# LeiXu84/fireFoam-dev

Measured on AMD Instinct MI355X. Metric: PIMPLE outer-iterations/sec on 64M-cell hex mesh; pEqn SpMV GB/s vs HBM peak, higher is better.
Workload: dtype f64; 1 GPU; synthetic 400^3 hex box (64000000 cells), buoyant plume + 5-species EDC-shaped source, PIMPLE 1/2/0: rhoEqn + UEqn + YEEqn(4 Yi + h) + 2 pEqn per step; cells=64000000, faces=191520000, parallelism=1 GPU, transport_solvers=PBiCGStab+DILU

## Files before the change

firefoam-dev_amd/binding.py:

```python
import ctypes as C
import os
import re
import subprocess

import numpy as np

_HERE = os.path.dirname(os.path.abspath(__file__))
_ROOT = os.path.dirname(_HERE)
_SO = os.path.join(_HERE, "lib", "libffm.so")
_HDR = os.path.join(_ROOT, "include", "ffm.h")

SOLVERS = {"PCG": 0, "PBiCGStab": 1, "PBiCG": 2, "diagonal": 3, "smoothSolver": 4}
PRECONDS = {"none": 0, "DIC": 1, "DILU": 2, "GaussSeidel": 3, "symGaussSeidel": 4, "diagonal": 5}


class FfmError(RuntimeError):
    pass


class Perf(C.Structure):
    _fields_ = [("initialResidual", C.c_double), ("finalResidual", C.c_double),
                ("nIterations", C.c_int), ("converged", C.c_int), ("singular", C.c_int)]

    def as_dict(self):
# ... 69 lines not shown
        "ffm_ldu_bind_coeffs_native_d": ([vp, dp, dp, dp, C.c_int], C.c_int),
        "ffm_ldu_set_interfaces": ([vp, C.c_int, ip, C.POINTER(ip), C.POINTER(hp), C.POINTER(hp), ip], C.c_int),
        "ffm_ldu_set_global_cells": ([vp, C.c_long], C.c_int),
        "ffm_ldu_global_cells": ([vp], C.c_long),
        "ffm_spmv": ([vp, dp, dp], C.c_int),
        "ffm_tmul": ([vp, dp, dp], C.c_int),
        "ffm_sumA": ([vp, dp], C.c_int),
        "ffm_residual": ([vp, dp, dp, dp], C.c_int),
        "ffm_precond_setup": ([vp, C.c_int, dp], C.c_int),
        "ffm_precond_apply": ([vp, C.c_int, C.c_int, dp, dp], C.c_int),
        "ffm_precond_setup_multi": ([vp, C.c_int, C.c_int, C.POINTER(C.c_void_p), C.POINTER(C.c_void_p)], C.c_int),
        "ffm_ldu_tile_reach": ([vp, C.POINTER(C.c_int), C.POINTER(C.c_int), C.POINTER(C.c_int)], C.c_int),
        "ffm_gs_smooth": ([vp, C.c_int, C.c_int, dp, dp], C.c_int),
        "ffm_solve_d": ([vp, C.c_int, C.c_int, C.c_double, C.c_double, C.c_int, C.c_int, C.c_int, dp, dp,
                         C.POINTER(Perf)], C.c_int),
        "ffm_solve": ([vp, C.c_int, C.c_int, C.c_double, C.c_double, C.c_int, C.c_int, C.c_int, hp, hp,
                       C.POINTER(Perf)], C.c_int),
        "ffm_solve_multi_d": ([vp, C.c_int, C.c_int, C.c_int, C.c_double, C.c_double, C.c_int, C.c_int, C.POINTER(C.c_void_p), dp, dp,
                               C.POINTER(C.c_void_p), C.POINTER(C.c_void_p), C.POINTER(Perf)], C.c_int),
        "ffm_ldu_unbind_coeffs": ([vp], C.c_int),
        "ffm_ldu_offdiag_epoch": ([vp], C.c_ulong),
        "ffm_ldu_tile_coef_read": ([vp, C.c_int, hp], C.c_int),
        "ffm_ldu_tile_gathers": ([vp], C.c_long),
        "ffm_debug_pool_poison": ([vp, C.c_int], C.c_int),
        "ffm_bench_spmv": ([vp, dp, dp, C.c_int, hp], C.c_int),
        "ffm_bench_precond": ([vp, C.c_int, dp, dp, C.c_int, hp], C.c_int),
        "ffm_debug_set_sweep_ticket": ([vp, C.c_uint], C.c_int),
        "ffm_ldu_set_exchange_tags": ([vp, C.c_int, C.c_int, ip], C.c_int),
        "ffm_field_binary": ([vp, C.c_int, C.c_long, dp, dp, dp], C.c_int),
        "ffm_field_scalar": ([vp, C.c_int, C.c_long, dp, C.c_double, C.c_int, dp], C.c_int),
        "ffm_field_unary": ([vp, C.c_int, C.c_long, dp, dp], C.c_int),
        "ffm_field_eval": ([vp, C.c_long, C.c_int, C.POINTER(C.c_void_p), C.c_int, hp, C.c_int, C.POINTER(C.c_ushort), dp], C.c_int),
        "ffm_reduce_sum": ([vp, dp, C.c_long, hp], C.c_int),
        "ffm_reduce_min": ([vp, dp, C.c_long, hp], C.c_int),
        "ffm_reduce_max": ([vp, dp, C.c_long, hp], C.c_int),
        "ffm_reduce_dot": ([vp, dp, dp, C.c_long, hp], C.c_int),
        "ffm_reduce_summag": ([vp, dp, C.c_long, hp], C.c_int),
        "ffm_mesh_create": ([vp, hp, hp, hp, hp, hp, hp, C.c_int, ip, C.POINTER(ip), C.POINTER(hp), C.POINTER(hp), C.POINTER(vp)], C.c_int),
        "ffm_mesh_destroy": ([vp], C.c_int),
        "ffm_mesh_set_face_centres": ([vp, hp], C.c_int),
        "ffm_mesh_set_nonorth_correction": ([vp, hp], C.c_int),
        "ffm_pyro_create": ([vp, C.c_int, C.c_int, C.c_double, C.c_double, C.c_double, C.c_double, C.POINTER(vp)], C.c_int),
        "ffm_pyro_set_solids": ([vp, hp, hp], C.c_int),
        "ffm_pyro_set_reaction": ([vp, C.c_double, C.c_double, C.c_double, C.c_double], C.c_int),
        "ffm_pyro_step": ([vp, C.c_double, dp, C.c_int, C.c_double], C.c_int),
        "ffm_pyro_get": ([vp, C.c_char_p, hp], C.c_int),
# ... 484 lines not shown
        return m

    def bind_coeffs_native(self, diag, upper, lower=None, offDiagUnchanged=False):
        self._bound = (diag, upper, lower)
        _check(lib().ffm_ldu_bind_coeffs_native_d(self.h, C.c_void_p(diag.data_ptr()), C.c_void_p(upper.data_ptr()),
                                                  None if lower is None else C.c_void_p(lower.data_ptr()), 1 if offDiagUnchanged else 0),
               "ffm_ldu_bind_coeffs_native_d")
        return self

    def unbind_coeffs(self):
        _check(lib().ffm_ldu_unbind_coeffs(self.h), "ffm_ldu_unbind_coeffs")
        self._bound = None
        return self

    def tile_coef(self, which):
        self.ctx._ready()
        out = np.empty(3 * self.nOwned, np.float64)
        _check(lib().ffm_ldu_tile_coef_read(self.h, which, _hp(out)), "ffm_ldu_tile_coef_read")
        return out

    def tile_gathers(self):
        return int(lib().ffm_ldu_tile_gathers(self.h))

    @property
    def offdiag_epoch(self):
        return int(lib().ffm_ldu_offdiag_epoch(self.h))

    def debug_set_sweep_ticket(self, value):
        _check(lib().ffm_debug_set_sweep_ticket(self.h, int(value) & 0xFFFFFFFF), "ffm_debug_set_sweep_ticket")

    @property
    def native_order(self):
        return bool(lib().ffm_ldu_is_native_order(self.h))

    def cell_order(self):
        o = np.empty(self.nCells, np.int32)
        _check(lib().ffm_ldu_get_cell_order(self.h, _ip(o)), "ffm_ldu_get_cell_order")
        return o

    def set_coeffs(self, diag, upper, lower=None):
        T = self.ctx.torch
        if T.is_tensor(diag):
            self.ctx._ready()
            lo = None if lower is None else C.c_void_p(lower.data_ptr())
            _check(lib().ffm_ldu_set_coeffs_d(self.h, C.c_void_p(diag.data_ptr()), C.c_void_p(upper.data_ptr()), lo),
                   "ffm_ldu_set_coeffs_d")
# ... 574 lines not shown
```

firefoam-dev_amd/csrc/ffm_host.hpp:

```cpp
#pragma once
#include <ctime>
#include <cstdio>
#include <cstdlib>
#include <cstring>
#include <vector>
#include <thread>
#include <algorithm>

#include "../../include/ffm.h"

void ffm_set_error(const char *fmt, ...);

#define FFM_TRY(call)                                                            \
    do {                                                                         \
        int r_ = (call);                                                         \
        if (r_ != FFM_OK) return r_;                                             \
    } while (0)

template <class Fn> inline void ffm_parallel_for(long n, Fn fn, long serialBelow = 1L << 20)
{
    static const int nT = [] { const char *e = getenv("FFM_HOST_THREADS"); int t = e ? atoi(e) : (int)std::thread::hardware_concurrency(); return std::max(1, std::min(t, 16)); }();
    if (n < serialBelow || nT == 1) { fn(0L, n); return; }
    std::vector<std::thread> th;
    const long chunk = (n + nT - 1) / nT;
// ... 24 lines not shown
    std::vector<int> newToOldCell, oldToNewCell, newToOldFace;
    std::vector<int> l, u;
    std::vector<int> fwdLevelStart;
    std::vector<int> bwdLevelStart;
    std::vector<int> bwdOrder;
    bool identity = true;
    int mode = 0, nGroups = 0; bool bwdIsReverse = false;
    std::vector<int> levNew, blNew;
    std::vector<int> grpCell;
};
struct LduLayout {
    int nSlices = 0, upTotal = 0, loTotal = 0;
    int upWidthUniform = -1, loWidthUniform = -1, maxW = 0;
    int loShift = 4;
    std::vector<int> upOff, loOff;
    std::vector<int> upNbr, faceSrc;
    std::vector<int> loEnt;
    std::vector<int> callerToNative;
    std::vector<int> rowSched;
};
int ffm_ldu_analysis(int nOwn, int nGhost, int F, const int *l, const int *u, const int *groupHint, int forceMode, LduAnalysis &a);
int ffm_ldu_layout(const LduAnalysis &a, int nOwn, int nGhost, int F, LduLayout &L);
bool ffm_tile_feasible(int nOwn, int F, const int *l, const int *u);
```

firefoam-dev_amd/csrc/ffm_tile.hip:

```cpp
#include "ffm_internal.hpp"
#include "ffm_device.hpp"
#include <algorithm>
#include <atomic>
#include <climits>

constexpr int T_RING = 4096;
constexpr int T_ENT = 256;
constexpr int T_THREADS = 256;
constexpr int T_W = FFM_TILE_W;
constexpr int T_PF = 8;
constexpr int T_PM = 3;
constexpr int T_XMAX = 64;
constexpr int T_RINGD = T_RING - 2 * T_ENT;
constexpr unsigned T_SPIN_LIMIT = 1u << 22;
constexpr unsigned T_NONE = 0xFFFFu;
constexpr int T_LDS = T_RING + 2 * T_XMAX + 1;
constexpr unsigned long long T_SENT = 0x7FF4DEADBEEFCAFEull;
static_assert(T_LDS < (int)T_NONE && T_ENT <= 256, "neighbour codes are LDS slots");
static_assert(T_PM >= 2 && T_PM < T_PF, "read-ahead distances");

struct TileDir {
    int nEnt = 0, nPub = 0;
    int *grpEnt = nullptr;
    int4 *rec = nullptr;
    int *extSrc = nullptr;
    unsigned short *code = nullptr;
    int *src = nullptr;
    double *coefU = nullptr, *coefL = nullptr;
    unsigned long epochU = ~0ul, epochL = ~0ul;
    int reach = 0;
    double *mail = nullptr;
};

struct ffm_tile_plan {
    bool usable = false;
    int G = 0;
    TileDir f, b;
    double *mailAll = nullptr;
    long nMail = 0;
    double *mailMulti = nullptr;
    bool amulUsable = false;
    bool gsTables = false;
    std::vector<int> grpEntHost;
    int4 *arec = nullptr;
    uint4 *acode = nullptr;
    int2 *aext = nullptr;
    int *upNbrCell = nullptr;
    int nSeg = 0;
    int4 *aseg = nullptr;
    double *amulPartials = nullptr;
    int4 *fvSeg = nullptr; int nFvSeg = 0, fvRun = 0;
    int nTail = 0;
    int *tailCell = nullptr, *tailStart = nullptr, *tailFace = nullptr, *tailNbr = nullptr;
};

bool ffm_tile_fv_segments(ffm_ldu *A, int runLength, FfmFvSegs *out)
{
    ffm_tile_plan *T = A->tile;
    if (!T || !T->usable || T->grpEntHost.empty() || A->nCells != A->nOwned) return false;
    if (!T->fvSeg || T->fvRun != runLength) {
        std::vector<int4> seg;
        const std::vector<int> &ge = T->grpEntHost;
        for (int g = 0; g < T->G; g++) for (int a = ge[g]; a < ge[g + 1]; a += runLength) seg.push_back(make_int4(ge[g], a, std::min(a + runLength, ge[g + 1]), ge[g + 1]));
        if (T->fvSeg) { hipFree(T->fvSeg); T->fvSeg = nullptr; }
        if (ffm_upload_vec(A->ctx, &T->fvSeg, seg) != FFM_OK) return false;
        T->nFvSeg = (int)seg.size(); T->fvRun = runLength;
    }
    out->nSeg = T->nFvSeg; out->seg = T->fvSeg; out->rec = T->f.rec;
    return true;
}

static void free_dir(TileDir &d)
{
    hipFree(d.grpEnt); hipFree(d.rec); hipFree(d.extSrc); hipFree(d.code); hipFree(d.src); hipFree(d.coefU); hipFree(d.coefL);
    d = TileDir();
}
void ffm_tile_free(ffm_ldu *A)
{
    if (!A->tile) return;
    free_dir(A->tile->f); free_dir(A->tile->b);
    hipFree(A->tile->mailAll); hipFree(A->tile->mailMulti);
    hipFree(A->tile->arec); hipFree(A->tile->acode); hipFree(A->tile->aext); hipFree(A->tile->aseg); hipFree(A->tile->amulPartials);
    hipFree(A->tile->fvSeg); hipFree(A->tile->upNbrCell);
    hipFree(A->tile->tailCell); hipFree(A->tile->tailStart); hipFree(A->tile->tailFace); hipFree(A->tile->tailNbr);
    delete A->tile; A->tile = nullptr;
}
bool ffm_tile_usable(const ffm_ldu *A) { return A->tile && A->tile->usable; }

template <class T> static int upv(ffm_ctx *c, T **d, const std::vector<T> &v) { return ffm_upload_vec(c, d, v); }

static int build_dir(ffm_ldu *A, bool fwd, const std::vector<int> &lvl, const std::vector<int> &grpCell,
                     const std::vector<int> &grpOfCell, TileDir &D, bool &ok, std::vector<int4> *recOut = nullptr,
                     std::vector<int> *grpEntOut = nullptr)
{
    const int G = (int)grpCell.size() - 1, nOwn = A->nOwned, W = T_W, sh = A->loShift;
    const std::vector<int> &off = fwd ? A->h_loOff : A->h_upOff;
    const std::vector<int> &ent = fwd ? A->h_loEnt : A->h_upNbr;
    std::vector<int> nbr((size_t)W * nOwn, -1), src((size_t)W * nOwn, -1);
    std::vector<unsigned char> exposed(nOwn, 0);
    auto isExt = [&](int c, int nb) { return grpOfCell[nb] != grpOfCell[c] || std::abs(c - nb) > T_RINGD; };
    std::atomic<int> tooMany(0), reach(0);
    ffm_parallel_for(nOwn, [&](long c0_, long c1_) {
        int far = 0;
        for (long c = c0_; c < c1_; c++) {
            const int sl = (int)(c >> 6), lane = (int)(c & 63), wdt = (off[sl + 1] - off[sl]) / 64;
            int k = 0;
            for (int s = 0; s < wdt; s++) {
                const int q = off[sl] + s * 64 + lane, e = ent[q];
                if (e < 0) continue;
                const int nb = fwd ? (e >> sh) : e;
                if (nb >= nOwn) continue;
                if (k >= W) { tooMany = 1; break; }
// ... 45 lines not shown
    for (int4 &R : rec) { R.w = (int)nExtAll; nExtAll += (size_t)(R.y >> 16); }
    std::vector<int> extSrc(nExtAll);
    std::atomic<int> bad(0);
    ffm_parallel_for((long)rec.size(), [&](long e0_, long e1_) {
        for (long ei = e0_; ei < e1_; ei++) {
            const int4 &R = rec[ei];
            const int c0 = R.x, cnt = R.y & 0xFFFF;
            const int gs = cnt ? grpCell[grpOfCell[c0]] : 0;
            int t = 0;
            for (int c = c0; c < c0 + cnt; c++) for (int k = 0; k < W; k++) {
                const int nb = nbr[(size_t)W * c + k];
                if (nb < 0) continue;
                if (isExt(c, nb)) {
                    if (mailIdx[nb] < 0 || t >= (R.y >> 16)) { bad = mailIdx[nb] < 0 ? 1 : 2; continue; }
                    code[(size_t)4 * c + k] = (unsigned short)(T_RING + (int)(ei & 1) * T_XMAX + t); extSrc[(size_t)R.w + t] = mailIdx[nb]; t++;
                } else code[(size_t)4 * c + k] = (unsigned short)((nb - gs) & (T_RING - 1));
            }
            if (t != (R.y >> 16)) bad = 2;
        }
    }, nOwn >= (1 << 20) ? 1024 : (1L << 40));
    if (bad == 1) { ffm_set_error("internal: tile plan references an unpublished cell"); return FFM_ERR_ADDR; }
    if (bad) { ffm_set_error("internal: tile plan external count mismatch"); return FFM_ERR_ADDR; }
    D.nEnt = (int)rec.size(); D.nPub = nPub;
    if (recOut) *recOut = rec;
    if (grpEntOut) *grpEntOut = grpEnt;
    for (int k = 0; k < 2 * T_PF + 2; k++) rec.push_back(make_int4(0, 0, 0, 0));
    for (int k = 0; k < T_THREADS; k++) extSrc.push_back(0);
    FFM_TRY(upv(A->ctx, &D.grpEnt, grpEnt)); FFM_TRY(upv(A->ctx, &D.rec, rec)); FFM_TRY(upv(A->ctx, &D.extSrc, extSrc)); FFM_TRY(upv(A->ctx, &D.code, code)); FFM_TRY(upv(A->ctx, &D.src, src));
    return FFM_OK;
}

constexpr int A_RING = 1024;
constexpr int A_WIN = 1;
constexpr int A_AHEAD = A_WIN + 1;
constexpr int A_XMAX = 128;
constexpr int A_PF = 6;
constexpr unsigned A_NONE = 0xFFFFu, A_EXT = 0x8000u;
static_assert((A_WIN + A_AHEAD + 1) * T_ENT <= A_RING && A_PF > A_AHEAD, "ring window");

static int build_amul(ffm_ldu *A, const std::vector<int> &grpOfCell, const std::vector<int4> &recF)
{
    ffm_tile_plan *T = A->tile;
    const int nOwn = A->nOwned, nEnt = (int)recF.size();
    std::vector<int> tailCell, tailStart(1, 0), tailFace, tailNbr;
    std::vector<int> upNb((size_t)3 * nOwn, -1);
    for (int c = 0; c < nOwn; c++) {
        const int sl = c >> 6, lane = c & 63;
        const int uw = (A->h_upOff[sl + 1] - A->h_upOff[sl]) / 64;
        int k = 0;
        bool ghostSeen = false;
        for (int s = 0; s < uw; s++) {
// ... 35 lines not shown
                const int o = q >> A->loShift, os = q & ((1 << A->loShift) - 1);
                if (k >= 3) { AMUL_GIVE_UP("more than 3 lower neighbours"); }
                if (inRing(c, o) && os < 3 && c - o < 2048) code[(size_t)8 * c + k] = (unsigned short)((c - o) | (os << 12));
                else {
                    if (t >= A_XMAX) { AMUL_GIVE_UP("more than A_XMAX externals in one entry"); }
                    code[(size_t)8 * c + k] = (unsigned short)(A_EXT | t);
                    aext.push_back(make_int2(o, A->h_upOff[o >> 6] + os * 64 + (o & 63))); t++;
                }
                k++;
            }
            for (k = 0; k < 3; k++) {
                const int nb = upNb[(size_t)3 * c + k];
                if (nb < 0) break;
                if (inRing(c, nb) && nb - c < 2048) code[(size_t)8 * c + 3 + k] = (unsigned short)(nb - c);
                else {
                    if (t >= A_XMAX) { AMUL_GIVE_UP("more than A_XMAX externals in one entry"); }
                    code[(size_t)8 * c + 3 + k] = (unsigned short)(A_EXT | t);
                    aext.push_back(make_int2(nb, -1)); t++;
                }
            }
        }
        arec[e] = make_int4(c0, cnt | (t << 16), extOff, 0);
    }
    for (int k = 0; k < 2 * A_PF + 2; k++) arec.push_back(make_int4(0, 0, 0, 0));
    for (int k = 0; k < 2 * A_XMAX; k++) aext.push_back(make_int2(0, -1));
    FFM_TRY(upv(A->ctx, &T->arec, arec)); FFM_TRY(upv(A->ctx, &T->aext, aext));
    FFM_HIP(hipMalloc((void **)&T->acode, sizeof(unsigned short) * 8 * std::max<size_t>(nOwn, 1)));
    FFM_TRY(ffm_h2d(A->ctx, T->acode, code.data(), sizeof(unsigned short) * code.size()));
    {
        const std::vector<int> &grpEntH = T->grpEntHost;
        const int L = std::min(20, std::max(16, nEnt / 2048));
        std::vector<int4> seg;
        for (int g = 0; g < T->G; g++) for (int a = grpEntH[g]; a < grpEntH[g + 1]; a += L) seg.push_back(make_int4(g, a, std::min(a + L, grpEntH[g + 1]), grpEntH[g + 1]));
        T->nSeg = (int)seg.size();
        FFM_TRY(upv(A->ctx, &T->aseg, seg));
        FFM_HIP(hipMalloc((void **)&T->amulPartials, sizeof(double) * std::max(T->nSeg, 1)));
    }
    T->amulUsable = true;
    return FFM_OK;
}

int ffm_tile_build(ffm_ldu *A, const std::vector<int> &lev, const std::vector<int> &bl, const std::vector<int> &grpCell)
{
    A->tile = new ffm_tile_plan();
    ffm_tile_plan *T = A->tile;
    T->G = (int)grpCell.size() - 1;
    if (T->G <= 0) return FFM_OK;
    const int nOwn = A->nOwned;
    if ((long)A->nCells * 24 >= (1L << 32)) return FFM_OK;
    std::vector<int> grpOfCell(nOwn);
    for (int g = 0; g < T->G; g++) for (int c = grpCell[g]; c < grpCell[g + 1]; c++) grpOfCell[c] = g;
    bool ok = true;
    std::vector<int4> recF;
    { FfmStageTimer tm_("tile: forward plan"); FFM_TRY(build_dir(A, true, lev, grpCell, grpOfCell, T->f, ok, &recF, &T->grpEntHost)); }
    if (ok) { FfmStageTimer tm_("tile: backward plan"); FFM_TRY(build_dir(A, false, bl, grpCell, grpOfCell, T->b, ok)); }
    T->usable = ok;
    if (ok) {
        T->nMail = (long)T->f.nPub + T->b.nPub + 2;
        FFM_HIP(hipMalloc((void **)&T->mailAll, sizeof(double) * T->nMail));
        T->f.mail = T->mailAll; T->b.mail = T->mailAll + T->f.nPub + 1;
        FfmStageTimer tm_("tile: amul plan");
        FFM_TRY(build_amul(A, grpOfCell, recF));
        if (!T->gsTables) T->usable = false;
    }
    return FFM_OK;
}

struct TileView {
    int G;
    const int *grpCell, *grpEnt, *extSrc;
    const int4 *rec;
    const uint2 *code;
    unsigned int *ticket;
};

__device__ __forceinline__ double t_ld(const double *p) { return __hip_atomic_load(p, __ATOMIC_RELAXED, __HIP_MEMORY_SCOPE_AGENT); }
__device__ __forceinline__ void t_st(double *p, double v) { __hip_atomic_store(p, v, __ATOMIC_RELAXED, __HIP_MEMORY_SCOPE_AGENT); }
__device__ __forceinline__ void t_barrier() { asm volatile("s_waitcnt lgkmcnt(0)\n\ts_barrier" ::: "memory"); }
__device__ __forceinline__ bool t_pending(double v) { return (unsigned long long)__double_as_longlong(v) == T_SENT; }

enum { TM_FWD = 0, TM_BWD = 1, TM_RD = 2, TM_GSF = 3, TM_GSB = 4 };
struct __attribute__((aligned(8))) T3 { double a, b, c; };
static_assert(T_W == 3, "T3");

__device__ __noinline__ double t_wait_value(const double *addr, unsigned int *ticket, int *shAbort)
{
    double v = t_ld(addr);
    if (*(volatile int *)shAbort) return v;
    unsigned spins = 0;
    while (t_pending(v)) {
        __builtin_amdgcn_s_sleep(1);
        v = t_ld(addr);
        if ((++spins & 1023u) == 0u) {
// ... 24 lines not shown
    constexpr bool VEC = MODE != TM_RD;
    constexpr int W = T_W, PF = tile_pf(NF, MODE);
    __shared__ double ring[NF][LDS];
    __shared__ double shSum[4];
    __shared__ int4 shRec[4];
    __shared__ int shG;
    __shared__ int shAbort;
    const unsigned tid = threadIdx.x;
    if (tid == 0) {
        const unsigned tk = atomicAdd(&t.ticket[0], 1u);
        const int k = (int)(tk % (unsigned)t.G);
        shG = ASC ? k : t.G - 1 - k; shAbort = 0;
    }
    __syncthreads();
    const int g = __builtin_amdgcn_readfirstlane(shG);
    const unsigned gs = (unsigned)__builtin_amdgcn_readfirstlane(t.grpCell[g]);
    const int e0 = __builtin_amdgcn_readfirstlane(t.grpEnt[g]), e1 = __builtin_amdgcn_readfirstlane(t.grpEnt[g + 1]);
    if (e0 >= e1) { if (FUSE && tid == 0) partials[g] = 0.0; return; }

    if (tid >= (unsigned)T_THREADS) {
        const unsigned lane = tid - (unsigned)T_THREADS;
        int4 qrec[PF];
        unsigned qne[PF], qxi[PF];
        double qxv[PF][NF];
#define Q_REC(k, e) { qrec[k] = t.rec[min((e), e1)]; }
#define Q_IDX(k, e) { const int4 R_ = qrec[k]; qne[k] = ((e) < e1) ? ((unsigned)R_.y >> 16) : 0u; qxi[k] = (unsigned)t.extSrc[(unsigned)R_.w + (lane < qne[k] ? lane : 0u)]; }
#define Q_MAIL(k) { _Pragma("unroll") for (int i_ = 0; i_ < NF; i_++) qxv[k][i_] = t_ld(&m.mail[i_][lane < qne[k] ? qxi[k] : 0u]); }
#define Q_PUT(k, e) {                                                                                    \
        if (lane < qne[k]) {                                                                              \
            _Pragma("unroll") for (int i_ = 0; i_ < NF; i_++) {                                           \
                double v_ = qxv[k][i_];                                                                   \
                if (__builtin_expect(t_pending(v_), 0)) v_ = t_wait_value(&m.mail[i_][qxi[k]], t.ticket, &shAbort); \
                ring[i_][R + (((e) & 1) * T_XMAX) + lane] = v_;                                           \
            }                                                                                             \
        }                                                                                                 \
    }
#pragma unroll
        for (int k = 0; k < PF; k++) Q_REC(k, e0 + k);
#pragma unroll
        for (int k = 0; k < PF; k++) { Q_IDX(k, e0 + k); Q_REC(k, e0 + PF + k); }
#pragma unroll
        for (int k = 0; k < T_PM; k++) Q_MAIL(k);
        Q_PUT(0, e0);
        if (lane == 0) shRec[(e0 + PF) & 3] = qrec[0];
        t_barrier();
        for (int e = e0; e < e1; e += PF) {
#pragma unroll
            for (int k = 0; k < PF; k++) {
                const int ee = e + k;
// ... 2 lines not shown
                Q_IDX(k, ee + PF);
                Q_REC(k, ee + 2 * PF);
                Q_MAIL((k + T_PM) % PF);
                t_barrier();
            }
        }
#undef Q_REC
#undef Q_IDX
#undef Q_MAIL
#undef Q_PUT
        return;
    }

    unsigned pc[PF], ppb[PF];
    bool pok[PF];
    uint2 pq[PF];
    double pa[PF][W], pb[PF][TWO ? W : 1], pd[PF][NF], pv[PF][VEC ? NF : 1], pv2[FUSE ? PF : 1];
    double fsum = 0.0;
    const double fAlpha = (FUSE && MODE == TM_FWD) ? scal[S_ALPHA] : 0.0;
    const bool fSing = (FUSE && MODE == TM_FWD) ? (scal[S_SING] != 0.0) : false;
#define T_FETCH(k, e, R_) {                                                                             \
        const unsigned cnt_ = ((e) < e1) ? ((unsigned)R_.y & 0xFFFFu) : 0u;                              \
        const bool ok_ = tid < cnt_;                                                                     \
        const unsigned cc_ = ok_ ? (ASC ? (unsigned)R_.x + tid : (unsigned)R_.x + cnt_ - 1u - tid) : gs; \
        const unsigned o8_ = cc_ * 8u, o24_ = cc_ * 24u;          \
        pq[k] = *(const uint2 *)((const char *)t.code + o8_);                                            \
        { const T3 v_ = *(const T3 *)((const char *)ca + o24_); pa[k][0] = v_.a; pa[k][1] = v_.b; pa[k][2] = v_.c; }     \
        if (TWO) { const T3 v_ = *(const T3 *)((const char *)cb + o24_); pb[k][0] = v_.a; pb[k][TWO ? 1 : 0] = v_.b; pb[k][TWO ? 2 : 0] = v_.c; } \
        _Pragma("unroll") for (int i_ = 0; i_ < NF; i_++) {                                              \
            pd[k][i_] = *(const double *)((const char *)m.dg[i_] + o8_);                                 \
            if (VEC) pv[k][VEC ? i_ : 0] = *(const double *)((const char *)((FUSE && MODE == TM_FWD) ? (const double *)aux : MODE == TM_BWD ? (const double *)m.w[i_] : m.r[i_]) + o8_); \
        }                                                                                                \
        if (FUSE) pv2[FUSE ? k : 0] = *(const double *)((const char *)((MODE == TM_FWD && !m.r[0]) ? (const double *)m.w[0] : m.r[0]) + o8_); \
        pc[k] = cc_; pok[k] = ok_; ppb[k] = (unsigned)R_.z;                                              \
    }
#pragma unroll
    for (int k = 0; k < PF; k++) { const int4 R0 = t.rec[min(e0 + k, e1)]; T_FETCH(k, e0 + k, R0); }
    t_barrier();
    for (int e = e0; e < e1; e += PF) {
#pragma unroll
        for (int k = 0; k < PF; k++) {
            const int ee = e + k;
            const int4 Rn = shRec[(ee + PF) & 3];
            {
                const unsigned c = pc[k];
                const unsigned cd[4] = {pq[k].x & 0xFFFFu, pq[k].x >> 16, pq[k].y & 0xFFFFu, pq[k].y >> 16};
                unsigned sl[W];
#pragma unroll
                for (int s = 0; s < W; s++)
// ... 68 lines not shown
    constexpr int W = T_W;
    constexpr int PF = tile_pf(1, MODE);
    __shared__ double ring[T_LDS];
    double *const halo = ring + T_RING;
    __shared__ int4 shRec[4];
    __shared__ int shG;
    __shared__ int shAbort;
    const unsigned tid = threadIdx.x;
    if (tid == 0) {
        const unsigned tk = atomicAdd(&t.ticket[0], 1u);
        const int k = (int)(tk % (unsigned)t.G);
        shG = ASC ? k : t.G - 1 - k; shAbort = 0;
    }
    __syncthreads();
    const int g = __builtin_amdgcn_readfirstlane(shG);
    const unsigned gs = (unsigned)__builtin_amdgcn_readfirstlane(t.grpCell[g]);
    const int e0 = __builtin_amdgcn_readfirstlane(t.grpEnt[g]), e1 = __builtin_amdgcn_readfirstlane(t.grpEnt[g + 1]);
    if (e0 >= e1) return;

    if (tid >= (unsigned)T_THREADS) {
        const unsigned lane = tid - (unsigned)T_THREADS;
        int4 qrec[PF];
        unsigned qne[PF], qxi[PF];
        double qxv[PF];
#define Q_REC(k, e) { qrec[k] = t.rec[min((e), e1)]; }
#define Q_IDX(k, e) { const int4 R_ = qrec[k]; qne[k] = ((e) < e1) ? ((unsigned)R_.y >> 16) : 0u; qxi[k] = (unsigned)t.extSrc[(unsigned)R_.w + (lane < qne[k] ? lane : 0u)]; }
#define Q_MAIL(k) { qxv[k] = t_ld(&mail[lane < qne[k] ? qxi[k] : 0u]); }
#define Q_PUT(k, e) {                                                                                    \
        if (lane < qne[k]) {                                                                              \
            double v_ = qxv[k];                                                                           \
            if (__builtin_expect(t_pending(v_), 0)) v_ = t_wait_value(&mail[qxi[k]], t.ticket, &shAbort); \
            halo[(((e) & 1) * T_XMAX) + lane] = v_;                                                       \
        }                                                                                                 \
    }
#pragma unroll
        for (int k = 0; k < PF; k++) Q_REC(k, e0 + k);
#pragma unroll
        for (int k = 0; k < PF; k++) { Q_IDX(k, e0 + k); Q_REC(k, e0 + PF + k); }
#pragma unroll
        for (int k = 0; k < T_PM; k++) Q_MAIL(k);
        Q_PUT(0, e0);
        if (lane == 0) shRec[(e0 + PF) & 3] = qrec[0];
        t_barrier();
        for (int e = e0; e < e1; e += PF) {
#pragma unroll
            for (int k = 0; k < PF; k++) {
                const int ee = e + k;
                Q_PUT((k + 1) % PF, ee + 1);
                if (lane == 0) shRec[(ee + 1 + PF) & 3] = qrec[(k + 1) % PF];
                Q_IDX(k, ee + PF);
                Q_REC(k, ee + 2 * PF);
                Q_MAIL((k + T_PM) % PF);
                t_barrier();
            }
        }
#undef Q_REC
#undef Q_IDX
#undef Q_MAIL
#undef Q_PUT
        return;
    }

    unsigned pc[PF], ppb[PF];
    bool pok[PF];
    uint2 pq[PF];
    double pa[PF][W], pb[PF][TWO ? W : 1], pd[PF], pv[PF];
#define T_FETCH(k, e, R_) {                                                                             \
        const unsigned cnt_ = ((e) < e1) ? ((unsigned)R_.y & 0xFFFFu) : 0u;                              \
        const bool ok_ = tid < cnt_;                                                                     \
        const unsigned cc_ = ok_ ? (ASC ? (unsigned)R_.x + tid : (unsigned)R_.x + cnt_ - 1u - tid) : gs; \
        const unsigned o8_ = cc_ * 8u, o24_ = cc_ * 24u;          \
        pq[k] = *(const uint2 *)((const char *)t.code + o8_);                                            \
        { const T3 v_ = *(const T3 *)((const char *)ca + o24_); pa[k][0] = v_.a; pa[k][1] = v_.b; pa[k][2] = v_.c; }     \
        if (TWO) { const T3 v_ = *(const T3 *)((const char *)cb + o24_); pb[k][0] = v_.a; pb[k][TWO ? 1 : 0] = v_.b; pb[k][TWO ? 2 : 0] = v_.c; } \
        pd[k] = *(const double *)((const char *)dg + o8_);                                               \
        pv[k] = *(const double *)((const char *)r + o8_);                                                \
        pc[k] = cc_; pok[k] = ok_; ppb[k] = (unsigned)R_.z;                                              \
    }
#pragma unroll
    for (int k = 0; k < PF; k++) { const int4 R0 = t.rec[min(e0 + k, e1)]; T_FETCH(k, e0 + k, R0); }
    t_barrier();
    for (int e = e0; e < e1; e += PF) {
#pragma unroll
        for (int k = 0; k < PF; k++) {
            const int ee = e + k;
            const int4 Rn = shRec[(ee + PF) & 3];
            {
                const unsigned c = pc[k];
                const unsigned cd[4] = {pq[k].x & 0xFFFFu, pq[k].x >> 16, pq[k].y & 0xFFFFu, pq[k].y >> 16};
                double x[W];
#pragma unroll
                for (int s = 0; s < W; s++) x[s] = ring[min(cd[s], (unsigned)(T_LDS - 1))];
                const double d = pd[k];
                double val;
                if (MODE == TM_GSF) {
// ... 15 lines not shown
            }
            T_FETCH(k, ee + PF, Rn);
            t_barrier();
        }
    }
#undef T_FETCH
}

__global__ void k_tile_gather(long n, const int *__restrict__ src, const double *__restrict__ native, double *__restrict__ out)
{
    for (long i = (long)blockIdx.x * blockDim.x + threadIdx.x; i < n; i += (long)gridDim.x * blockDim.x) {
        const int q = src[i];
        out[i] = (q >= 0) ? native[q] : 0.0;
    }
}
__global__ void k_tile_fill(long n, unsigned long long *p, unsigned long long v, unsigned int *ticket)
{
    if (blockIdx.x == 0 && threadIdx.x == 0) ticket[0] = 0u;
    for (long i = (long)blockIdx.x * blockDim.x + threadIdx.x; i < n; i += (long)gridDim.x * blockDim.x) p[i] = v;
}

static TileView tview(const ffm_ldu *A, const TileDir &d)
{
    TileView t; t.G = A->tile->G; t.grpCell = A->grpCell; t.grpEnt = d.grpEnt; t.extSrc = d.extSrc; t.rec = d.rec;
    t.code = (const uint2 *)d.code; t.ticket = A->sweepTicket;
    return t;
}

static int tile_coef(ffm_ldu *A, TileDir &d, bool upper, const double **out)
{
    const long n = (long)T_W * A->nOwned;
    double *&buf = upper ? d.coefU : d.coefL;
    unsigned long &ep = upper ? d.epochU : d.epochL;
    if (!buf) { FFM_HIP(hipMalloc((void **)&buf, sizeof(double) * std::max<long>(n, 1))); ep = ~0ul; }
    if (ep != A->offDiagEpoch) {
        const int g = std::max(1, std::min(ffm_grid(n, 256), 8 * RED_BLOCKS));
        hipLaunchKernelGGL(k_tile_gather, dim3(g), dim3(256), 0, A->ctx->stream, n, d.src, upper ? A->upper : A->lower, buf);
        ep = A->offDiagEpoch;
        A->tileGathers++;
    }
    *out = buf;
    return FFM_OK;
}

bool ffm_tile_coef_direct_ok(const ffm_ldu *A) { return ffm_tile_usable(A) && A->nCells == A->nOwned && A->maxW <= T_W && A->identity; }
int ffm_tile_coef_direct(ffm_ldu *A, bool lower, double **fU, double **fL, double **bU)
{
// ... 10 lines not shown
    A->directPending = false;
    *fU = T->f.coefU; *fL = lower ? T->f.coefL : nullptr; *bU = T->b.coefU;
    return FFM_OK;
}
void ffm_tile_coef_written(ffm_ldu *A, const double *upper_d, const double *lower_d)
{
    A->directPending = true; A->directUpper = upper_d; A->directLower = (lower_d && lower_d != upper_d) ? lower_d : nullptr;
}
void ffm_tile_coef_adopt(ffm_ldu *A)
{
    ffm_tile_plan *T = A->tile;
    T->f.epochU = T->b.epochU = A->offDiagEpoch;
    if (A->directLower) T->f.epochL = A->offDiagEpoch;
}
extern "C" int ffm_ldu_tile_coef_read(ffm_ldu *A, int which, double *out_h)
{
    if (!A || !out_h || which < 0 || which > 3) return FFM_ERR_ARG;
    if (!ffm_tile_usable(A)) { ffm_set_error("ffm_ldu_tile_coef_read: the matrix has no tile plan"); return FFM_ERR_UNSUPPORTED; }
    const double *p;
    FFM_TRY(tile_coef(A, which < 2 ? A->tile->f : A->tile->b, !(which & 1), &p));
    return ffm_d2h(A->ctx, out_h, p, sizeof(double) * (size_t)T_W * A->nOwned);
}
extern "C" long ffm_ldu_tile_gathers(const ffm_ldu *A) { return A ? (long)A->tileGathers : -1; }

static void tile_fill(ffm_ldu *A, double *p, long n)
{
    const int g = std::max(1, std::min(ffm_grid(n, 256), 8 * RED_BLOCKS));
    hipLaunchKernelGGL(k_tile_fill, dim3(g), dim3(256), 0, A->ctx->stream, n, (unsigned long long *)p, T_SENT, A->sweepTicket);
}

bool ffm_tile_multi_fits(const ffm_ldu *A, int n)
{
    if (n < 1 || n > FFM_TILE_MAXSYS || !ffm_tile_usable(A)) return false;
    return n <= 4 || std::max(A->tile->f.reach, A->tile->b.reach) <= TM_RING5 - 2 * T_ENT;
}
extern "C" int ffm_ldu_tile_reach(const ffm_ldu *A, int *reach, int *limit, int *limit5)
{
    if (!A || !reach || !limit || !limit5) return FFM_ERR_ARG;
    if (!ffm_tile_usable(A)) { ffm_set_error("ffm_ldu_tile_reach: the matrix has no tile plan"); return FFM_ERR_UNSUPPORTED; }
    *reach = std::max(A->tile->f.reach, A->tile->b.reach); *limit = T_RINGD; *limit5 = TM_RING5 - 2 * T_ENT;
    return FFM_OK;
}
static int tile_mail(ffm_ldu *A, int n, bool fwdOnly, double **mail)
{
    ffm_tile_plan *T = A->tile;
    if (n > 1 && !T->mailMulti) FFM_HIP(hipMalloc((void **)&T->mailMulti, sizeof(double) * (size_t)FFM_TILE_MAXSYS * (size_t)T->nMail));
// ... 164 lines not shown
                    if (lane == 0) shRec[(ee + 1 + A_PF) & 3] = qrec[(k + 1) % A_PF];
                    Q_IDX(k, ee + A_PF);
                    Q_REC(k, ee + 2 * A_PF);
                    Q_VAL((k + T_PM) % A_PF);
                    t_barrier();
                }
            }
#undef Q_REC
#undef Q_IDX
#undef Q_VAL
#undef Q_PUT
#undef Q_X0
#undef Q_X1
        } else {
            unsigned pc[A_PF];
            bool pok[A_PF], pst[A_PF];
            uint4 pq[A_PF];
            double pb[A_PF][3], pd[A_PF], px[A_PF], pp[FUSEP ? A_PF : 1], ps[FUSEP ? A_PF : 1], pl[ASYM ? A_PF : 1][3];
#define A_FETCH(k, e, R_) {                                                                              \
        const unsigned cnt_ = ((e) < e1) ? ((unsigned)(R_).y & 0xFFFFu) : 0u;                            \
        const bool ok_ = tid < cnt_;                                                                     \
        const unsigned cc_ = ok_ ? (unsigned)(R_).x + tid : gs;                                          \
        const unsigned o8_ = cc_ * 8u;                                                                   \
        pq[k] = *(const uint4 *)((const char *)t.code + cc_ * 16u);                                      \
        { const T3 v_ = *(const T3 *)((const char *)bc + cc_ * 24u); pb[k][0] = v_.a; pb[k][1] = v_.b; pb[k][2] = v_.c; } \
        pd[k] = *(const double *)((const char *)diag + o8_);                                             \
        px[k] = *(const double *)((const char *)x + o8_);                                                \
        if (FUSEP) { pp[FUSEP ? k : 0] = *(const double *)((const char *)pin + o8_); ps[FUSEP ? k : 0] = *(const double *)((const char *)psi + o8_); } \
        if (ASYM) { const T3 v_ = *(const T3 *)((const char *)lc + cc_ * 24u); pl[ASYM ? k : 0][0] = v_.a; pl[ASYM ? k : 0][1] = v_.b; pl[ASYM ? k : 0][2] = v_.c; } \
        pc[k] = cc_; pok[k] = ok_; pst[k] = ok_ && (e) >= sa && (e) < sb;                                \
    }
#define A_FILL(k) { if (FUSEP) px[k] = fSing ? pp[FUSEP ? k : 0] : px[k] + fBeta * pp[FUSEP ? k : 0];                      \
                    if (pok[k]) { const unsigned i_ = (pc[k] - gs) & (unsigned)(A_RING - 1); xring[i_] = px[k];    \
                                   cring[3u * i_] = pb[k][0]; cring[3u * i_ + 1u] = pb[k][1]; cring[3u * i_ + 2u] = pb[k][2]; } }
#pragma unroll
            for (int k = 0; k < A_PF; k++) { const int4 R0 = t.rec[min(e0 + k, e1)]; A_FETCH(k, e0 + k, R0); }
#pragma unroll
            for (int k = 0; k < A_AHEAD; k++) A_FILL(k);
            t_barrier();
            for (int e = e0; e < sb; e += A_PF) {
#pragma unroll
                for (int k = 0; k < A_PF; k++) {
                    const int ee = e + k;
                    const int4 Rn = shRec[(ee + A_PF) & 3];
                    {
                        const unsigned c = pc[k];
                        const unsigned hb = (unsigned)(ee & 1) * (unsigned)A_XMAX;
// ... 157 lines not shown
```

include/ffm.h:

```cpp
#ifndef FFM_H
#define FFM_H

#include <stddef.h>
#include <stdint.h>

#ifdef __cplusplus
extern "C" {
#endif

typedef struct ffm_ctx ffm_ctx;
typedef struct ffm_ldu ffm_ldu;

typedef enum ffm_status {
    FFM_OK = 0,
    FFM_ERR_ARG = -1,
    FFM_ERR_ADDR = -2,
    FFM_ERR_HIP = -3,
    FFM_ERR_NODEVICE = -4,
    FFM_ERR_UNSUPPORTED = -5,
    FFM_ERR_COMM = -6
} ffm_status;

typedef enum ffm_solver {
    FFM_PCG = 0, FFM_PBICGSTAB = 1, FFM_PBICG = 2, FFM_DIAGONAL = 3, FFM_SMOOTH = 4,
// ... 62 lines not shown
int ffm_ldu_sweep_mode(const ffm_ldu *ldu);
int ffm_ldu_is_native_order(const ffm_ldu *ldu);
int ffm_ldu_get_cell_order(const ffm_ldu *ldu, int *newToOld);

int ffm_renumber_levels(int nCells, int nFaces, const int *lowerAddr,
                        const int *upperAddr, int *newToOldCell,
                        int *newToOldFace);

int ffm_ldu_set_coeffs(ffm_ldu *ldu, const double *diag, const double *upper,
                       const double *lower);
int ffm_ldu_set_coeffs_d(ffm_ldu *ldu, const double *diag_d,
                         const double *upper_d, const double *lower_d);

int ffm_ldu_n_native_faces(const ffm_ldu *ldu);
int ffm_ldu_get_face_map(const ffm_ldu *ldu, int *callerToNative);
int ffm_ldu_set_coeffs_native_d(ffm_ldu *ldu, const double *diag_d,
                                const double *upper_d, const double *lower_d);
int ffm_ldu_bind_coeffs_native_d(ffm_ldu *ldu, const double *diag_d, const double *upper_d,
                                 const double *lower_d, int offDiagUnchanged);
int ffm_ldu_unbind_coeffs(ffm_ldu *ldu);
unsigned long ffm_ldu_offdiag_epoch(const ffm_ldu *ldu);
int ffm_ldu_tile_coef_read(ffm_ldu *ldu, int which, double *out_h);
long ffm_ldu_tile_gathers(const ffm_ldu *ldu);

int ffm_ldu_set_interfaces(ffm_ldu *ldu, int nPatches, const int *patchSizes,
                           const int *const *faceCells,
                           const double *const *bouCoeffs,
                           const double *const *intCoeffs,
                           const int *neighbRank);
int ffm_ldu_set_global_cells(ffm_ldu *ldu, long globalCells);
long ffm_ldu_global_cells(const ffm_ldu *ldu);
int ffm_ldu_set_exchange_tags(ffm_ldu *ldu, int kind, int n, const int *tags);

int ffm_spmv(ffm_ldu *ldu, const double *x_d, double *y_d);
int ffm_tmul(ffm_ldu *ldu, const double *x_d, double *y_d);
int ffm_sumA(ffm_ldu *ldu, double *s_d);
int ffm_residual(ffm_ldu *ldu, const double *x_d, const double *b_d, double *r_d);
int ffm_precond_setup(ffm_ldu *ldu, int precond, double *rD_out_d );
int ffm_precond_apply(ffm_ldu *ldu, int precond, int transpose,
                      const double *r_d, double *w_d);
int ffm_precond_setup_multi(ffm_ldu *ldu, int precond, int nSys, const double *const *diag_d, double *const *rD_out_d);
int ffm_ldu_tile_reach(const ffm_ldu *ldu, int *reach, int *limit, int *limit5);
int ffm_gs_smooth(ffm_ldu *ldu, int symmetric_sweep, int nSweeps, double *psi_d,
                  const double *b_d);

int ffm_solve_d(ffm_ldu *ldu, int solver, int precond, double tolerance,
// ... 365 lines not shown
```

Measured before the change: 3.308 outer-iterations/s.

## Deduplicate per-tile neighbour code blocks into a shared pool

Hashes each tile entry's neighbour-code block at setup and stores identical blocks once in a shared pool, with each record's w field now holding a byte offset into that pool. The external-source offset that used to live in rec.w moves to a separate extOff array. On a structured hex box many tiles have identical connectivity codes, so code reads in the sweep and amul kernels can hit a much smaller, cache-resident footprint. The cost is an extra extOff load per entry, an indirect code address, and host-side hashing at setup; it can be turned off with FFM_TILE_CODE_SHARE.

```diff
diff --git a/firefoam-dev_amd/binding.py b/firefoam-dev_amd/binding.py
--- a/firefoam-dev_amd/binding.py
+++ b/firefoam-dev_amd/binding.py
@@ -115,6 +115,9 @@
         "ffm_ldu_offdiag_epoch": ([vp], C.c_ulong),
         "ffm_ldu_tile_coef_read": ([vp, C.c_int, hp], C.c_int),
         "ffm_ldu_tile_gathers": ([vp], C.c_long),
+        "ffm_ldu_tile_code_bytes": ([vp, C.c_int, C.POINTER(C.c_long), C.POINTER(C.c_long)], C.c_int),
+        "ffm_tile_share_codes": ([C.c_int, C.POINTER(C.c_long), ip, C.POINTER(C.c_ushort), C.c_long, C.c_int, C.c_long, C.POINTER(C.c_uint),
+                                  C.POINTER(C.c_ushort), C.c_long, C.POINTER(C.c_long), C.POINTER(C.c_long)], C.c_int),
         "ffm_debug_pool_poison": ([vp, C.c_int], C.c_int),
         "ffm_bench_spmv": ([vp, dp, dp, C.c_int, hp], C.c_int),
         "ffm_bench_precond": ([vp, C.c_int, dp, dp, C.c_int, hp], C.c_int),
@@ -645,6 +648,11 @@
     def tile_gathers(self):
         return int(lib().ffm_ldu_tile_gathers(self.h))
 
+    def tile_code_bytes(self, which):
+        u, t = C.c_long(), C.c_long()
+        _check(lib().ffm_ldu_tile_code_bytes(self.h, which, C.byref(u), C.byref(t)), "ffm_ldu_tile_code_bytes")
+        return u.value, t.value
+
     @property
     def offdiag_epoch(self):
         return int(lib().ffm_ldu_offdiag_epoch(self.h))
diff --git a/firefoam-dev_amd/csrc/ffm_host.hpp b/firefoam-dev_amd/csrc/ffm_host.hpp
--- a/firefoam-dev_amd/csrc/ffm_host.hpp
+++ b/firefoam-dev_amd/csrc/ffm_host.hpp
@@ -70,3 +70,7 @@
 int ffm_ldu_analysis(int nOwn, int nGhost, int F, const int *l, const int *u, const int *groupHint, int forceMode, LduAnalysis &a);
 int ffm_ldu_layout(const LduAnalysis &a, int nOwn, int nGhost, int F, LduLayout &L);
 bool ffm_tile_feasible(int nOwn, int F, const int *l, const int *u);
+
+int ffm_tile_share(std::vector<unsigned short> &codes, const std::vector<long> &start, const std::vector<int> &len, bool share, long padShorts,
+                   std::vector<unsigned short> &pool, std::vector<unsigned> &off, long *uniqueBytes, long *totalBytes, const char *what);
+bool ffm_tile_share_enabled(int reader);
diff --git a/firefoam-dev_amd/csrc/ffm_tile.hip b/firefoam-dev_amd/csrc/ffm_tile.hip
--- a/firefoam-dev_amd/csrc/ffm_tile.hip
+++ b/firefoam-dev_amd/csrc/ffm_tile.hip
@@ -23,8 +23,10 @@
     int nEnt = 0, nPub = 0;
     int *grpEnt = nullptr;
     int4 *rec = nullptr;
+    int *extOff = nullptr;
     int *extSrc = nullptr;
     unsigned short *code = nullptr;
+    long codeUnique = 0, codeTotal = 0;
     int *src = nullptr;
     double *coefU = nullptr, *coefL = nullptr;
     unsigned long epochU = ~0ul, epochL = ~0ul;
@@ -44,6 +46,7 @@
     std::vector<int> grpEntHost;
     int4 *arec = nullptr;
     uint4 *acode = nullptr;
+    long acodeUnique = 0, acodeTotal = 0;
     int2 *aext = nullptr;
     int *upNbrCell = nullptr;
     int nSeg = 0;
@@ -72,7 +75,7 @@
 
 static void free_dir(TileDir &d)
 {
-    hipFree(d.grpEnt); hipFree(d.rec); hipFree(d.extSrc); hipFree(d.code); hipFree(d.src); hipFree(d.coefU); hipFree(d.coefL);
+    hipFree(d.grpEnt); hipFree(d.rec); hipFree(d.extOff); hipFree(d.extSrc); hipFree(d.code); hipFree(d.src); hipFree(d.coefU); hipFree(d.coefL);
     d = TileDir();
 }
 void ffm_tile_free(ffm_ldu *A)
@@ -88,6 +91,18 @@
 bool ffm_tile_usable(const ffm_ldu *A) { return A->tile && A->tile->usable; }
 
 template <class T> static int upv(ffm_ctx *c, T **d, const std::vector<T> &v) { return ffm_upload_vec(c, d, v); }
+
+static int share_blocks(std::vector<unsigned short> &code, std::vector<int4> &rec, int S, const char *what, std::vector<unsigned short> &pool,
+                        long *uniqueBytes, long *totalBytes, std::vector<int> *wOut)
+{
+    std::vector<long> start(rec.size());
+    std::vector<int> len(rec.size());
+    for (size_t e = 0; e < rec.size(); e++) { start[e] = (long)S * rec[e].x; len[e] = S * (rec[e].y & 0xFFFF); }
+    std::vector<unsigned> off;
+    FFM_TRY(ffm_tile_share(code, start, len, ffm_tile_share_enabled(S == 4 ? 1 : 2), (long)S * T_ENT, pool, off, uniqueBytes, totalBytes, what));
+    for (size_t e = 0; e < rec.size(); e++) { if (wOut) (*wOut)[e] = rec[e].w; rec[e].w = (int)off[e]; }
+    return FFM_OK;
+}
 
 static int build_dir(ffm_ldu *A, bool fwd, const std::vector<int> &lvl, const std::vector<int> &grpCell,
                      const std::vector<int> &grpOfCell, TileDir &D, bool &ok, std::vector<int4> *recOut = nullptr,
@@ -179,11 +194,15 @@
     if (bad == 1) { ffm_set_error("internal: tile plan references an unpublished cell"); return FFM_ERR_ADDR; }
     if (bad) { ffm_set_error("internal: tile plan external count mismatch"); return FFM_ERR_ADDR; }
     D.nEnt = (int)rec.size(); D.nPub = nPub;
+    std::vector<int> extOff(rec.size());
+    std::vector<unsigned short> pool;
+    FFM_TRY(share_blocks(code, rec, 4, fwd ? "tile: forward code sharing" : "tile: backward code sharing", pool, &D.codeUnique, &D.codeTotal, &extOff));
     if (recOut) *recOut = rec;
     if (grpEntOut) *grpEntOut = grpEnt;
-    for (int k = 0; k < 2 * T_PF + 2; k++) rec.push_back(make_int4(0, 0, 0, 0));
+    for (int k = 0; k < 2 * T_PF + 2; k++) { rec.push_back(make_int4(0, 0, 0, 0)); extOff.push_back(0); }
     for (int k = 0; k < T_THREADS; k++) extSrc.push_back(0);
-    FFM_TRY(upv(A->ctx, &D.grpEnt, grpEnt)); FFM_TRY(upv(A->ctx, &D.rec, rec)); FFM_TRY(upv(A->ctx, &D.extSrc, extSrc)); FFM_TRY(upv(A->ctx, &D.code, code)); FFM_TRY(upv(A->ctx, &D.src, src));
+    FFM_TRY(upv(A->ctx, &D.grpEnt, grpEnt)); FFM_TRY(upv(A->ctx, &D.rec, rec)); FFM_TRY(upv(A->ctx, &D.extOff, extOff)); FFM_TRY(upv(A->ctx, &D.extSrc, extSrc));
+    FFM_TRY(upv(A->ctx, &D.code, pool)); FFM_TRY(upv(A->ctx, &D.src, src));
     return FFM_OK;
 }
 
@@ -265,11 +284,13 @@
         }
         arec[e] = make_int4(c0, cnt | (t << 16), extOff, 0);
     }
+    std::vector<unsigned short> pool;
+    FFM_TRY(share_blocks(code, arec, 8, "tile: amul code sharing", pool, &T->acodeUnique, &T->acodeTotal, nullptr));
     for (int k = 0; k < 2 * A_PF + 2; k++) arec.push_back(make_int4(0, 0, 0, 0));
     for (int k = 0; k < 2 * A_XMAX; k++) aext.push_back(make_int2(0, -1));
     FFM_TRY(upv(A->ctx, &T->arec, arec)); FFM_TRY(upv(A->ctx, &T->aext, aext));
-    FFM_HIP(hipMalloc((void **)&T->acode, sizeof(unsigned short) * 8 * std::max<size_t>(nOwn, 1)));
-    FFM_TRY(ffm_h2d(A->ctx, T->acode, code.data(), sizeof(unsigned short) * code.size()));
+    FFM_HIP(hipMalloc((void **)&T->acode, sizeof(unsigned short) * pool.size()));
+    FFM_TRY(ffm_h2d(A->ctx, T->acode, pool.data(), sizeof(unsigned short) * pool.size()));
     {
         const std::vector<int> &grpEntH = T->grpEntHost;
         const int L = std::min(20, std::max(16, nEnt / 2048));
@@ -311,7 +332,7 @@
 
 struct TileView {
     int G;
-    const int *grpCell, *grpEnt, *extSrc;
+    const int *grpCell, *grpEnt, *extOff, *extSrc;
     const int4 *rec;
     const uint2 *code;
     unsigned int *ticket;
@@ -382,9 +403,10 @@
         const unsigned lane = tid - (unsigned)T_THREADS;
         int4 qrec[PF];
         unsigned qne[PF], qxi[PF];
+        unsigned qxo[PF];
         double qxv[PF][NF];
-#define Q_REC(k, e) { qrec[k] = t.rec[min((e), e1)]; }
-#define Q_IDX(k, e) { const int4 R_ = qrec[k]; qne[k] = ((e) < e1) ? ((unsigned)R_.y >> 16) : 0u; qxi[k] = (unsigned)t.extSrc[(unsigned)R_.w + (lane < qne[k] ? lane : 0u)]; }
+#define Q_REC(k, e) { const int e_ = min((e), e1); qrec[k] = t.rec[e_]; qxo[k] = (unsigned)t.extOff[e_]; }
+#define Q_IDX(k, e) { const int4 R_ = qrec[k]; qne[k] = ((e) < e1) ? ((unsigned)R_.y >> 16) : 0u; qxi[k] = (unsigned)t.extSrc[qxo[k] + (lane < qne[k] ? lane : 0u)]; }
 #define Q_MAIL(k) { _Pragma("unroll") for (int i_ = 0; i_ < NF; i_++) qxv[k][i_] = t_ld(&m.mail[i_][lane < qne[k] ? qxi[k] : 0u]); }
 #define Q_PUT(k, e) {                                                                                    \
         if (lane < qne[k]) {                                                                              \
@@ -433,9 +455,10 @@
 #define T_FETCH(k, e, R_) {                                                                             \
         const unsigned cnt_ = ((e) < e1) ? ((unsigned)R_.y & 0xFFFFu) : 0u;                              \
         const bool ok_ = tid < cnt_;                                                                     \
-        const unsigned cc_ = ok_ ? (ASC ? (unsigned)R_.x + tid : (unsigned)R_.x + cnt_ - 1u - tid) : gs; \
+        const unsigned ps_ = ok_ ? (ASC ? tid : cnt_ - 1u - tid) : 0u;       \
+        const unsigned cc_ = ok_ ? (unsigned)R_.x + ps_ : gs;                                            \
         const unsigned o8_ = cc_ * 8u, o24_ = cc_ * 24u;          \
-        pq[k] = *(const uint2 *)((const char *)t.code + o8_);                                            \
+        pq[k] = *(const uint2 *)((const char *)t.code + ((unsigned)R_.w + ps_ * 8u));                    \
         { const T3 v_ = *(const T3 *)((const char *)ca + o24_); pa[k][0] = v_.a; pa[k][1] = v_.b; pa[k][2] = v_.c; }     \
         if (TWO) { const T3 v_ = *(const T3 *)((const char *)cb + o24_); pb[k][0] = v_.a; pb[k][TWO ? 1 : 0] = v_.b; pb[k][TWO ? 2 : 0] = v_.c; } \
         _Pragma("unroll") for (int i_ = 0; i_ < NF; i_++) {                                              \
@@ -550,9 +573,10 @@
         const unsigned lane = tid - (unsigned)T_THREADS;
         int4 qrec[PF];
         unsigned qne[PF], qxi[PF];
+        unsigned qxo[PF];
         double qxv[PF];
-#define Q_REC(k, e) { qrec[k] = t.rec[min((e), e1)]; }
-#define Q_IDX(k, e) { const int4 R_ = qrec[k]; qne[k] = ((e) < e1) ? ((unsigned)R_.y >> 16) : 0u; qxi[k] = (unsigned)t.extSrc[(unsigned)R_.w + (lane < qne[k] ? lane : 0u)]; }
+#define Q_REC(k, e) { const int e_ = min((e), e1); qrec[k] = t.rec[e_]; qxo[k] = (unsigned)t.extOff[e_]; }
+#define Q_IDX(k, e) { const int4 R_ = qrec[k]; qne[k] = ((e) < e1) ? ((unsigned)R_.y >> 16) : 0u; qxi[k] = (unsigned)t.extSrc[qxo[k] + (lane < qne[k] ? lane : 0u)]; }
 #define Q_MAIL(k) { qxv[k] = t_ld(&mail[lane < qne[k] ? qxi[k] : 0u]); }
 #define Q_PUT(k, e) {                                                                                    \
         if (lane < qne[k]) {                                                                              \
@@ -596,9 +620,10 @@
 #define T_FETCH(k, e, R_) {                                                                             \
         const unsigned cnt_ = ((e) < e1) ? ((unsigned)R_.y & 0xFFFFu) : 0u;                              \
         const bool ok_ = tid < cnt_;                                                                     \
-        const unsigned cc_ = ok_ ? (ASC ? (unsigned)R_.x + tid : (unsigned)R_.x + cnt_ - 1u - tid) : gs; \
+        const unsigned ps_ = ok_ ? (ASC ? tid : cnt_ - 1u - tid) : 0u;       \
+        const unsigned cc_ = ok_ ? (unsigned)R_.x + ps_ : gs;                                            \
         const unsigned o8_ = cc_ * 8u, o24_ = cc_ * 24u;          \
-        pq[k] = *(const uint2 *)((const char *)t.code + o8_);                                            \
+        pq[k] = *(const uint2 *)((const char *)t.code + ((unsigned)R_.w + ps_ * 8u));                    \
         { const T3 v_ = *(const T3 *)((const char *)ca + o24_); pa[k][0] = v_.a; pa[k][1] = v_.b; pa[k][2] = v_.c; }     \
         if (TWO) { const T3 v_ = *(const T3 *)((const char *)cb + o24_); pb[k][0] = v_.a; pb[k][TWO ? 1 : 0] = v_.b; pb[k][TWO ? 2 : 0] = v_.c; } \
         pd[k] = *(const double *)((const char *)dg + o8_);                                               \
@@ -660,7 +685,7 @@
 
 static TileView tview(const ffm_ldu *A, const TileDir &d)
 {
-    TileView t; t.G = A->tile->G; t.grpCell = A->grpCell; t.grpEnt = d.grpEnt; t.extSrc = d.extSrc; t.rec = d.rec;
+    TileView t; t.G = A->tile->G; t.grpCell = A->grpCell; t.grpEnt = d.grpEnt; t.extOff = d.extOff; t.extSrc = d.extSrc; t.rec = d.rec;
     t.code = (const uint2 *)d.code; t.ticket = A->sweepTicket;
     return t;
 }
@@ -717,6 +742,15 @@
     return ffm_d2h(A->ctx, out_h, p, sizeof(double) * (size_t)T_W * A->nOwned);
 }
 extern "C" long ffm_ldu_tile_gathers(const ffm_ldu *A) { return A ? (long)A->tileGathers : -1; }
+extern "C" int ffm_ldu_tile_code_bytes(const ffm_ldu *A, int which, long *uniqueBytes, long *totalBytes)
+{
+    if (!A || !uniqueBytes || !totalBytes || which < 0 || which > 2) return FFM_ERR_ARG;
+    if (!ffm_tile_usable(A)) { ffm_set_error("ffm_ldu_tile_code_bytes: the matrix has no tile plan"); return FFM_ERR_UNSUPPORTED; }
+    const ffm_tile_plan *T = A->tile;
+    *uniqueBytes = which == 0 ? T->f.codeUnique : which == 1 ? T->b.codeUnique : T->acodeUnique;
+    *totalBytes = which == 0 ? T->f.codeTotal : which == 1 ? T->b.codeTotal : T->acodeTotal;
+    return FFM_OK;
+}
 
 static void tile_fill(ffm_ldu *A, double *p, long n)
 {
@@ -927,7 +961,7 @@
         const bool ok_ = tid < cnt_;                                                                     \
         const unsigned cc_ = ok_ ? (unsigned)(R_).x + tid : gs;                                          \
         const unsigned o8_ = cc_ * 8u;                                                                   \
-        pq[k] = *(const uint4 *)((const char *)t.code + cc_ * 16u);                                      \
+        pq[k] = *(const uint4 *)((const char *)t.code + ((unsigned)(R_).w + (ok_ ? tid : 0u) * 16u));      \
         { const T3 v_ = *(const T3 *)((const char *)bc + cc_ * 24u); pb[k][0] = v_.a; pb[k][1] = v_.b; pb[k][2] = v_.c; } \
         pd[k] = *(const double *)((const char *)diag + o8_);                                             \
         px[k] = *(const double *)((const char *)x + o8_);                                                \
diff --git a/firefoam-dev_amd/csrc/ffm_tile_share.cpp b/firefoam-dev_amd/csrc/ffm_tile_share.cpp
--- /dev/null
+++ b/firefoam-dev_amd/csrc/ffm_tile_share.cpp
@@ -0,0 +1,90 @@
+#include "ffm_host.hpp"
+#include <cstdint>
+#include <unordered_map>
+
+static inline uint64_t share_hash(const unsigned short *p, size_t n)
+{
+    uint64_t h = 0x9E3779B97F4A7C15ull * (uint64_t)(n + 1);
+    size_t i = 0;
+    for (; i + 4 <= n; i += 4) { uint64_t w; memcpy(&w, p + i, 8); h = (h ^ w) * 0xFF51AFD7ED558CCDull; h ^= h >> 29; }
+    for (; i < n; i++) { h = (h ^ p[i]) * 0xC4CEB9FE1A85EC53ull; h ^= h >> 31; }
+    return h;
+}
+
+int ffm_tile_share(std::vector<unsigned short> &codes, const std::vector<long> &start, const std::vector<int> &len, bool share, long padShorts,
+                   std::vector<unsigned short> &pool, std::vector<unsigned> &off, long *uniqueBytes, long *totalBytes, const char *what)
+{
+    FfmStageTimer tm_(what ? what : "tile: code sharing");
+    const long nB = (long)start.size();
+    long total = 0;
+    for (long i = 0; i < nB; i++) {
+        if (len[i] < 0 || start[i] < 0 || start[i] + len[i] > (long)codes.size()) { ffm_set_error("internal: code block %ld outside the code array", i); return FFM_ERR_ARG; }
+        total += len[i];
+    }
+    off.assign(nB, 0u);
+    pool.clear();
+    long unique = 0;
+    if (!share) {
+        pool.swap(codes);
+        for (long i = 0; i < nB; i++) off[i] = len[i] ? (unsigned)(2 * start[i]) : 0u;
+        unique = total;
+        if (2 * (long)pool.size() + 2 * padShorts >= (1L << 32)) { ffm_set_error("tile plan: neighbour codes of 4 GiB or more"); return FFM_ERR_UNSUPPORTED; }
+    } else {
+        std::vector<uint64_t> hash(nB);
+        ffm_parallel_for(nB, [&](long a, long b) { for (long i = a; i < b; i++) hash[i] = share_hash(codes.data() + start[i], (size_t)len[i]); }, 4096);
+        std::unordered_map<uint64_t, long> head;
+        head.reserve((size_t)std::min<long>(nB, 1L << 16));
+        std::vector<long> next(nB, -1);
+        std::vector<long> poolAt(nB, -1);
+        for (long i = 0; i < nB; i++) {
+            if (!len[i]) continue;
+            const unsigned short *p = codes.data() + start[i];
+            auto it = head.find(hash[i]);
+            long rep = -1;
+            if (it != head.end())
+                for (long j = it->second; j >= 0; j = next[j])
+                    if (len[j] == len[i] && memcmp(pool.data() + poolAt[j], p, sizeof(unsigned short) * (size_t)len[i]) == 0) { rep = j; break; }
+            if (rep < 0) {
+                if (2 * ((long)pool.size() + len[i] + padShorts) >= (1L << 32)) { ffm_set_error("tile plan: neighbour codes of 4 GiB or more"); return FFM_ERR_UNSUPPORTED; }
+                poolAt[i] = (long)pool.size();
+                pool.insert(pool.end(), p, p + len[i]);
+                if (it != head.end()) { next[i] = it->second; it->second = i; } else head.emplace(hash[i], i);
+                rep = i;
+            }
+            off[i] = (unsigned)(2 * poolAt[rep]);
+        }
+        unique = (long)pool.size();
+        std::vector<unsigned short>().swap(codes);
+    }
+    pool.insert(pool.end(), (size_t)std::max<long>(padShorts, 0), (unsigned short)0xFFFFu);
+    if (uniqueBytes) *uniqueBytes = 2 * unique;
+    if (totalBytes) *totalBytes = 2 * total;
+    return FFM_OK;
+}
+
+bool ffm_tile_share_enabled(int reader)
+{
+    const char *e = getenv("FFM_TILE_CODE_SHARE");
+    const int mask = (e && *e) ? atoi(e) : 3;
+    return (mask & reader) != 0;
+}
+
+extern "C" int ffm_tile_share_codes(int nBlocks, const long *start, const int *len, const unsigned short *codes, long nCodes, int share, long padShorts,
+                                    unsigned int *offset_out, unsigned short *pool_out, long poolCapacity, long *uniqueShorts, long *poolShorts)
+{
+    if (nBlocks < 0 || nCodes < 0 || padShorts < 0 || (nBlocks && (!start || !len || !offset_out)) || (nCodes && !codes) || !uniqueShorts || !poolShorts) {
+        ffm_set_error("ffm_tile_share_codes: bad argument");
+        return FFM_ERR_ARG;
+    }
+    std::vector<unsigned short> c(codes, codes + nCodes), pool;
+    std::vector<long> s(start, start + nBlocks);
+    std::vector<int> l(len, len + nBlocks);
+    std::vector<unsigned> off;
+    long ub = 0, tb = 0;
+    FFM_TRY(ffm_tile_share(c, s, l, share != 0, padShorts, pool, off, &ub, &tb, nullptr));
+    if ((long)pool.size() > poolCapacity || (pool.size() && !pool_out)) { ffm_set_error("ffm_tile_share_codes: the pool needs %ld shorts, %ld given", (long)pool.size(), poolCapacity); return FFM_ERR_ARG; }
+    if (!pool.empty()) memcpy(pool_out, pool.data(), sizeof(unsigned short) * pool.size());
+    for (int i = 0; i < nBlocks; i++) offset_out[i] = off[i];
+    *uniqueShorts = ub / 2; *poolShorts = (long)pool.size();
+    return FFM_OK;
+}
diff --git a/include/ffm.h b/include/ffm.h
--- a/include/ffm.h
+++ b/include/ffm.h
@@ -108,6 +108,9 @@
 unsigned long ffm_ldu_offdiag_epoch(const ffm_ldu *ldu);
 int ffm_ldu_tile_coef_read(ffm_ldu *ldu, int which, double *out_h);
 long ffm_ldu_tile_gathers(const ffm_ldu *ldu);
+int ffm_ldu_tile_code_bytes(const ffm_ldu *ldu, int which, long *uniqueBytes, long *totalBytes);
+int ffm_tile_share_codes(int nBlocks, const long *start, const int *len, const unsigned short *codes, long nCodes, int share, long padShorts,
+                         unsigned int *offset_out, unsigned short *pool_out, long poolCapacity, long *uniqueShorts, long *poolShorts);
 
 int ffm_ldu_set_interfaces(ffm_ldu *ldu, int nPatches, const int *patchSizes,
                            const int *const *faceCells,
```

Measured after the change: 3.417 outer-iterations/s (median of 6 runs). 3.3% higher.
